# kujason/monopsr

Hardware: AMD Instinct MI355X
Metric: instance-crops/sec (fwd+Chamfer) (higher is better)
Workload: dtype f32; 1 GPU; BASELINE cfg3: batch=256/GPU synthetic 48x48 crops -> ResNet-101 trunk(block3, os4) + squash/map-decoder/xyz + heads fwd, + 1024-pt nn_distance Chamfer fwd/bwd; batch_per_gpu=256, global_batch=256, points=1024, streams_per_gpu=1

## Files before the change

monopsr_amd/csrc/internal.h:

```cpp
#pragma once
#include <hip/hip_runtime.h>

#include <atomic>
#include <cstddef>

#include "monopsr_hip.h"

namespace mpsr {

char *error_buffer();
extern thread_local int t_call_math;
extern thread_local int t_call_wino_policy;

int conv2d(const float *x, int B, int H, int W, int C, const float *w, const float *bias, const float *residual,
           float *y, int N, int KH, int KW, int dilation, int relu, int split_k, float *ws, size_t ws_floats,
           hipStream_t stream);
size_t conv_scratch_floats(long long M, int N);
bool conv2d_takes_winograd4(int B, int H, int W, int C, int N, const float *ws, size_t ws_floats);
bool conv2d_takes_winograd3(int B, int H, int W, int C, int N, int KH, int KW, int dilation, int split_k, const float *ws,
                            size_t ws_floats);
bool conv2d_takes_pointwise(long long M, int C, int N, int KH, int KW, int split_k);
int conv2d_winograd_choice(int B, int H, int W, int C, int N, int KH, int KW, int dilation, bool residual, int split_k,
                           const float *ws, size_t ws_floats);

int conv3x3_narrow(const float *x, int B, int H, int W, int C, const float *w, const float *bias, int relu, float *y,
                   int N, hipStream_t s, int in_c8);
bool conv3x3_narrow_takes_mfma(const float *x, int B, int H, int W, int C, int N, const float *w);
int resize_bilinear_c8(const float *in, int B, int H, int W, int C, int OH, int OW, int align_corners, float *out,
                       hipStream_t s);

size_t winograd_scratch_floats(int C, int N);
bool winograd_applies(int H, int W, int C, int N);
bool winograd_applies_dilated(int H, int W, int C, int N, int dilation);
int conv3x3_winograd(const float *x, int B, int H, int W, int C, const float *w, const float *bias, int relu, float *y,
                     int N, float *ws, size_t ws_floats, hipStream_t s, int dilation);
extern std::atomic<int> g_wino_waves;

size_t winograd4_scratch_floats(int C, int N);
bool winograd4_applies(int H, int W, int C, int N);
int conv3x3_winograd4(const float *x, int B, int H, int W, int C, const float *w, const float *bias, int relu,
                      float *y, int N, float *ws, size_t ws_floats, hipStream_t s, int in_c8, int out_c8, float *part,
                      size_t part_floats);
size_t winograd4_split_floats(int B, int H, int W, int N);
extern std::atomic<int> g_wino4_split;

size_t winograd3_scratch_floats(int C, int N);
bool winograd3_applies(int H, int W, int C, int dilation);
double winograd3_executed_flops(int B, int H, int C, int N, int dilation);
int winograd3_form(int B, int H, int W, int C, int N, int dilation);
int winograd3_filter_form(int B, int H, int W, int C, int N, int dilation);
int conv3x3_winograd3(const float *x, int B, int H, int W, int C, const float *w, const float *bias, int relu,
                      float *y, int N, int dilation, float *ws, size_t ws_floats, hipStream_t s,
                      const float *mask = nullptr);
struct FilterTailJob {
    const float *w = nullptr;
    float *u = nullptr;
    int N = 0, C = 0;
    int form = 0;
};
extern thread_local FilterTailJob g_filter_tail_job;
extern thread_local FilterTailJob g_filter_tail_done;
struct FilterCacheSlot {
    const float *w = nullptr;
    float *u = nullptr;
    size_t floats = 0;
    bool ready = false;
    int *tag = nullptr;
    bool holds(int kind)
    {
        const bool ok = ready && (!tag || *tag == kind);
        if (tag) *tag = kind;
        return ok;
    }
};
enum { FILTER_FORM_WINO4 = 1, FILTER_FORM_WINO3 = 2, FILTER_FORM_UPCONV = 3, FILTER_FORM_WINO3Z = 4, FILTER_FORM_WINO2 = 5 };
extern thread_local FilterCacheSlot g_filter_cache_slot;

bool winograd3w_applies(int B, int H, int W, int C, int N, int dilation);
long long winograd3w_workgroups(int B, int N, int dilation);
int launch_winograd3w(const float *x, int B, int H, int W, int C, const float *u, const float *bias, int relu, float *y,
                      int N, int dilation, hipStream_t s, const float *mask);

// ... 42 lines not shown
```

monopsr_amd/csrc/network.hip:

```cpp
#include <atomic>
#include <vector>

#include "common.h"

static std::atomic<int> g_decoder_c8{1};
extern "C" void mpsr_debug_set_decoder_c8(int on) { g_decoder_c8 = on; }
static std::atomic<int> g_decoder_upconv{1};
extern "C" void mpsr_debug_set_decoder_upconv(int on) { g_decoder_upconv = on; }

namespace {

struct Arena {
    char *base;
    size_t size, used = 0;
    bool ok = true;
    Arena(void *p, size_t n) : base(static_cast<char *>(p)), size(n) {}
    float *floats(size_t n)
    {
        const size_t bytes = mpsr::align_up(n * sizeof(float), 256);
        if (used + bytes > size) {
            ok = false;
            return nullptr;
        }
        float *r = reinterpret_cast<float *>(base + used);
// ... 91 lines not shown
                              int n_layers, float *out, void *workspace, size_t workspace_bytes, mpsr_stream_t stream)
{
    return mpsr_trunk_fwd_ex(img, B, H, W, blob, layers, n_layers, out, workspace, workspace_bytes, nullptr, stream);
}

extern "C" int mpsr_trunk_fwd_ex(const float *img, int B, int H, int W, const float *blob, const mpsr_layer *layers,
                                 int n_layers, float *out, void *workspace, size_t workspace_bytes,
                                 const mpsr_net_opts *opts, mpsr_stream_t stream)
{
    MPSR_REQUIRE(B >= 0 && H >= 7 && W >= 7, "trunk_fwd: bad input shape (B=%d H=%d W=%d)", B, H, W);
    if (opts) {
        MPSR_REQUIRE(opts->math >= 0 && opts->math <= MPSR_CALL_MATH_BF16X3, "%s: unknown opts.math %d", "trunk_fwd", opts->math);
        MPSR_REQUIRE(opts->winograd_policy >= 0 && opts->winograd_policy <= MPSR_CALL_WINOGRAD_ACCURATE,
                     "%s: unknown opts.winograd_policy %d", "trunk_fwd", opts->winograd_policy);
    }
    mpsr::CallOptsGuard call_opts(opts ? opts->math : 0, opts ? opts->winograd_policy : 0);
    MPSR_REQUIRE(n_layers == MPSR_TRUNK_LAYERS, "trunk_fwd: expected %d layer records, got %d", MPSR_TRUNK_LAYERS,
                 n_layers);
    if (B == 0) return MPSR_OK;
    MPSR_REQUIRE(img && blob && layers && out && workspace, "trunk_fwd: null pointer");
    hipStream_t s = mpsr::as_stream(stream);
    const TrunkDims d = trunk_dims(H, W);
    const size_t Mr = (size_t)B * d.OH * d.OW, Mp = (size_t)B * d.PH * d.PW;
    const mpsr_layer &root = layers[0];
    MPSR_REQUIRE(root.kh == 1 && root.kw == 1 && root.cin >= 147 && root.cin % 32 == 0,
                 "trunk_fwd: layer 0 must be the root as a 1x1 layer over im2col columns (cin=%d)", root.cin);
    int cmax = 0, bmax = 0;
    for (int i = 1; i < n_layers; ++i) {
        if (layers[i].kh == 3 && layers[i].cout > bmax) bmax = layers[i].cout;
        if (layers[i].cout > cmax) cmax = layers[i].cout;
    }
    Arena ar(workspace, workspace_bytes);
    float *cols = ar.floats(Mr * root.cin);
    float *rootout = ar.floats(Mr * root.cout);
    float *pooled = ar.floats(Mp * root.cout);
    float *ping = ar.floats(Mp * cmax), *pong = ar.floats(Mp * cmax), *scut = ar.floats(Mp * cmax);
    float *t1 = ar.floats(Mp * bmax), *t2 = ar.floats(Mp * bmax);
    const size_t skn = mpsr::conv_scratch_floats((long long)(Mr > Mp ? Mr : Mp), cmax > 1024 ? cmax : 1024);
    float *sk = ar.floats(skn);
    if (!ar.ok)
        return mpsr::fail(MPSR_ERR_WORKSPACE, "trunk_fwd: workspace %zu bytes too small (see mpsr_trunk_workspace_bytes)",
                          workspace_bytes);

    int rc;
    struct TailJobGuard {
        ~TailJobGuard()
        {
            mpsr::g_filter_tail_job = mpsr::FilterTailJob();
            mpsr::g_filter_tail_done = mpsr::FilterTailJob();
            mpsr::g_filter_cache_slot = mpsr::FilterCacheSlot();
        }
    } tail_job_guard;
    FilterCache cache(opts);
    if ((rc = mpsr_im2col_root(img, B, H, W, cols, root.cin, stream))) return rc;
    if ((rc = run_layer(blob, root, cols, B, d.OH, d.OW, nullptr, rootout, 0, sk, skn, s))) return rc;
    if ((rc = mpsr_max_pool(rootout, B, d.OH, d.OW, root.cout, 3, 2, 1, pooled, stream))) return rc;

    const float *cur = pooled;
    int cur_c = root.cout;
    int li = 1;
    for (int blk = 0; blk < 3; ++blk) {
        for (int u = 0; u < kTrunkUnits[blk]; ++u) {
            const bool last = (blk == 2 && u == kTrunkUnits[blk] - 1);
            const float *residual = cur;
            if (u == 0) {
                const mpsr_layer &S = layers[li++];
                MPSR_REQUIRE(S.kh == 1 && S.cin == cur_c && !S.relu, "trunk_fwd: record %d is not a shortcut", li - 1);
                if ((rc = run_layer(blob, S, cur, B, d.PH, d.PW, nullptr, scut, 0, sk, skn, s))) return rc;
                residual = scut;
            }
            const mpsr_layer &c1 = layers[li], &c2 = layers[li + 1], &c3 = layers[li + 2];
            li += 3;
            MPSR_REQUIRE(c1.kh == 1 && c1.cin == cur_c && c2.kh == 3 && c2.cin == c1.cout && c3.kh == 1 &&
                             c3.cin == c2.cout && (u == 0 || c3.cout == cur_c),
                         "trunk_fwd: records %d..%d do not form a bottleneck unit", li - 3, li - 1);
            float *dst = last ? out : (cur == ping ? pong : ping);
            float *uslice = cache.take(c2);
            const int c2i = (int)(&c2 - layers);
            const int fform = mpsr::winograd3_filter_form(B, d.PH, d.PW, c2.cin, c2.cout, c2.dilation);
            const bool cached_u = uslice && cache.valid && (!cache.tags || cache.tags[c2i] == fform);
            if (!cached_u &&
                mpsr::conv2d_takes_pointwise((long long)B * d.PH * d.PW, c1.cin, c1.cout, 1, 1, 0) &&
                mpsr::conv2d_takes_winograd3(B, d.PH, d.PW, c2.cin, c2.cout, c2.kh, c2.kw, c2.dilation, 0, sk, skn)) {
                mpsr::g_filter_tail_job.w = blob + c2.w_off;
                mpsr::g_filter_tail_job.u = uslice ? uslice : sk;
                mpsr::g_filter_tail_job.N = c2.cout;
                mpsr::g_filter_tail_job.C = c2.cin;
                mpsr::g_filter_tail_job.form = fform == mpsr::FILTER_FORM_WINO3Z ? 1 : 0;
            }
            if ((rc = run_layer(blob, c1, cur, B, d.PH, d.PW, nullptr, t1, 0, sk, skn, s))) return rc;
            mpsr::g_filter_tail_job = mpsr::FilterTailJob();
            cache.offer(blob + c2.w_off, uslice, c2, c2i);
            rc = run_layer(blob, c2, t1, B, d.PH, d.PW, nullptr, t2, 0, sk, skn, s);
            mpsr::g_filter_cache_slot = mpsr::FilterCacheSlot();
            if (rc) return rc;
            if ((rc = run_layer(blob, c3, t2, B, d.PH, d.PW, residual, dst, 0, sk, skn, s))) return rc;
            cur = dst;
            cur_c = c3.cout;
        }
    }
    return MPSR_OK;
}


namespace {
struct DecoderChoice {
    bool c8, up1, up2, xyz_c8;
};
DecoderChoice decoder_choice(int B, int fh, int fw, int mh, int mw, const mpsr_layer *L, const float *blob, bool feat_map,
// ... 398 lines not shown
```

monopsr_amd/csrc/upconv.hip:

```cpp
#include <atomic>

#include "common.h"

namespace {

using f32x2 = __attribute__((ext_vector_type(2))) float;
using f32x4 = __attribute__((ext_vector_type(4))) float;
constexpr int PART = 1152;
constexpr size_t kGatherLdsBytes = 80 * 1024;

__global__ __launch_bounds__(256) void upconv_weights_kernel(const float *__restrict__ g, int N, int C, float *__restrict__ wp)
{
    const long long i = (long long)blockIdx.x * 256 + threadIdx.x;
    const int c4 = C / 4;
    if (i >= (long long)9 * N * c4) return;
    const int j = (int)(i / c4), q = (int)(i - (long long)j * c4);
    const int blk = j / 72, r = j - blk * 72, t = r >> 3, n = blk * 8 + (r & 7);
    reinterpret_cast<float4 *>(wp)[i] = reinterpret_cast<const float4 *>(g + ((size_t)n * 9 + t) * C)[q];
}

struct UpcParams {
    const float *z, *bias;
    float *y;
    size_t part_stride;
    int B, h, w, H, W, N, relu;
    int RB, cap;
    mpsr::FastDiv capdiv;
    float hscale, wscale;
};

constexpr int kPf = 8;
std::atomic<int> g_upconv_band{0};

template <bool OUT_C8>
__global__ __launch_bounds__(512) void upconv_gather_kernel(const UpcParams p)
{
    extern __shared__ __attribute__((aligned(16))) float4 src4[];
    const int tid = threadIdx.x, nthr = blockDim.x;
    const int nblk = p.N >> 3;
    const int xcd = blockIdx.x & 7, jx = blockIdx.x >> 3;
    const int bq = jx / nblk, blk = jx - bq * nblk, b = bq * 8 + xcd;
    if (b >= p.B) return;
    const int lpr = 2 * p.W, rpp = nthr / lpr;
    const int rr = tid / lpr, l = tid - rr * lpr, x = l >> 1, half = l & 1;
    const int n0 = blk * 8;
    const int rowf4 = p.w * 18;
    auto slot = [&](int r) __attribute__((always_inline)) { return r - p.cap * mpsr::fdiv(r, p.capdiv); };
    const float *zp = p.z + (size_t)(blk >> 4) * p.part_stride + (size_t)(blk & 15) * 72 + (size_t)b * p.h * p.w * PART;
    const int lgroups = nthr / 18, lgrp = tid / 18, lpiece = tid - lgrp * 18;
    const bool loader = lgrp < lgroups;
    const int lrow0 = lgrp / p.w, lcol0 = lgrp - lrow0 * p.w;
    const int drow = lgroups / p.w, dcol = lgroups - drow * p.w;
    f32x4 pf[kPf];
    auto issue = [&](int ra, int npix, int first) __attribute__((always_inline)) {
#pragma unroll
        for (int j = 0; j < kPf; ++j) {
            const int pix = first + lgrp + j * lgroups;
            const bool live = loader && pix < npix;
            pf[j] = *reinterpret_cast<const f32x4 *>(live ? zp + ((size_t)ra * p.w + pix) * PART + 4 * lpiece : zp);
        }
    };
    auto commit = [&](int ra, int npix, int first, int &row, int &col) __attribute__((always_inline)) {
#pragma unroll
        for (int j = 0; j < kPf; ++j) {
            const int pix = first + lgrp + j * lgroups;
            if (loader && pix < npix)
                reinterpret_cast<f32x4 *>(src4)[slot(ra + row) * rowf4 + col * 18 + lpiece] = pf[j];
            row += drow;
            col += dcol;
            if (col >= p.w) {
                col -= p.w;
                ++row;
            }
        }
    };

    auto band_rows = [&](int k, int &lo, int &hi) __attribute__((always_inline)) {
        const int y0 = k * p.RB, yl = min(y0 + p.RB, p.H) - 1;
        lo = (int)floorf((float)max(y0 - 1, 0) * p.hscale);
        hi = min((int)floorf((float)min(yl + 1, p.H - 1) * p.hscale) + 1, p.h - 1);
    };
    int co[3][2];
    float wx[3][2];
#pragma unroll
    for (int d = 0; d < 3; ++d) {
        const int qx = x + d - 1;
        const bool vx = qx >= 0 && qx < p.W;
        const float sx = (float)min(max(qx, 0), p.W - 1) * p.wscale;
        const int c0 = (int)floorf(sx), c1 = min(c0 + 1, p.w - 1);
        const float lx = sx - (float)c0;
        co[d][0] = c0 * 18 + half;
        co[d][1] = c1 * 18 + half;
        wx[d][0] = vx ? 1.f - lx : 0.f;
        wx[d][1] = vx ? lx : 0.f;
    }
    const float4 bias4 = p.bias ? *reinterpret_cast<const float4 *>(p.bias + n0 + 4 * half) : make_float4(0.f, 0.f, 0.f, 0.f);

    const int nbands = (p.H + p.RB - 1) / p.RB;
    int lo, hi;
    band_rows(0, lo, hi);
    {
        const int npix = (hi - lo + 1) * p.w;
        int row = lrow0, col = lcol0;
        for (int first = 0; first < npix; first += kPf * lgroups) {
            issue(lo, npix, first);
            commit(lo, npix, first, row, col);
        }
    }
    __syncthreads();
    for (int k = 0; k < nbands; ++k) {
        int nlo = 0, nhi = hi;
        if (k + 1 < nbands) band_rows(k + 1, nlo, nhi);
        const int nnew = (nhi - hi) * p.w;
        issue(hi + 1, nnew, 0);
        const int y0 = k * p.RB, ylast = min(y0 + p.RB, p.H) - 1;
        for (int y = y0 + rr; y <= ylast; y += rpp) {
            int ro[3][2];
            float wy[3][2];
#pragma unroll
            for (int d = 0; d < 3; ++d) {
                const int qy = y + d - 1;
                const bool vy = qy >= 0 && qy < p.H;
                const float sy = (float)min(max(qy, 0), p.H - 1) * p.hscale;
                const int r0 = (int)floorf(sy), r1 = min(r0 + 1, p.h - 1);
                const float ly = sy - (float)r0;
                ro[d][0] = slot(r0) * rowf4;
                ro[d][1] = slot(r1) * rowf4;
                wy[d][0] = vy ? 1.f - ly : 0.f;
                wy[d][1] = vy ? ly : 0.f;
            }
            f32x2 a01 = {bias4.x, bias4.y}, a23 = {bias4.z, bias4.w};
#pragma unroll
            for (int dy = 0; dy < 3; ++dy)
#pragma unroll
                for (int dx = 0; dx < 3; ++dx) {
                    const int t2 = 2 * (dy * 3 + dx);
#pragma unroll
                    for (int a = 0; a < 2; ++a)
#pragma unroll
                        for (int c = 0; c < 2; ++c) {
                            const float wgt = wy[dy][a] * wx[dx][c];
                            const float4 v = src4[ro[dy][a] + co[dx][c] + t2];
                            const f32x2 w2 = {wgt, wgt};
                            a01 = __builtin_elementwise_fma(w2, f32x2{v.x, v.y}, a01);
                            a23 = __builtin_elementwise_fma(w2, f32x2{v.z, v.w}, a23);
                        }
                }
            float4 acc = make_float4(a01.x, a01.y, a23.x, a23.y);
            if (p.relu) {
                acc.x = fmaxf(acc.x, 0.f);
                acc.y = fmaxf(acc.y, 0.f);
                acc.z = fmaxf(acc.z, 0.f);
                acc.w = fmaxf(acc.w, 0.f);
            }
            float *o = OUT_C8 ? p.y + ((((size_t)b * (p.N / 8) + blk) * p.H + y) * p.W + x) * 8 + 4 * half
                              : p.y + (((size_t)b * p.H + y) * p.W + x) * p.N + n0 + 4 * half;
            *reinterpret_cast<float4 *>(o) = acc;
        }
        if (k + 1 == nbands) break;
        __syncthreads();
        {
            int row = lrow0, col = lcol0;
            commit(hi + 1, nnew, 0, row, col);
        }
        __syncthreads();
        hi = nhi;
    }
}

constexpr int kGtMax = 8;
constexpr int kGtPf = 6;
constexpr int kGtItemsA = 6, kGtItemsB = 8;

struct UpcGradParams {
    const float *dy;
    float *dz;
    int B, h, w, H, W, N, rows_max, cap;
    float hscale, wscale;
};

__global__ __launch_bounds__(256) void upconv_gather_t_kernel(const UpcGradParams p)
{
    extern __shared__ __attribute__((aligned(16))) float4 g4[];
    const int tid = threadIdx.x;
    const int grp = blockIdx.x, b = blockIdx.y;
    const int rowq = p.W * 8;
    float4 *V = g4 + (size_t)p.cap * rowq;
    int *xq = reinterpret_cast<int *>(V + (size_t)3 * rowq);
    float *xw = reinterpret_cast<float *>(xq + p.w * kGtMax);
    int *xc = reinterpret_cast<int *>(xw + p.w * kGtMax);
    int *yq = xc + ((p.w + 3) & ~3);
    float *yw = reinterpret_cast<float *>(yq + p.h * kGtMax);
    int *yc = reinterpret_cast<int *>(yw + p.h * kGtMax);
    int *ylo = yc + p.h, *yhi = ylo + p.h;
    for (int t = tid; t < p.h + p.w; t += 256) {
        const bool row = t < p.h;
        const int sv = row ? t : t - p.h, n_in = row ? p.h : p.w, n_out = row ? p.H : p.W;
        const float scale = row ? p.hscale : p.wscale;
        const int q_lo = max((int)floorf((float)(sv - 1) / scale) - 1, 0), q_hi = min((int)ceilf((float)(sv + 1) / scale) + 1, n_out - 1);
        int *oq = row ? yq + sv * kGtMax : xq + sv * kGtMax;
        float *ow = row ? yw + sv * kGtMax : xw + sv * kGtMax;
        int c = 0, lo = n_out, hi = -1;
        for (int q = q_lo; q <= q_hi; ++q) {
            const float sq = (float)q * scale;
            const int r0 = (int)floorf(sq), r1 = min(r0 + 1, n_in - 1);
            const float l = sq - (float)r0;
            if ((r0 == sv || r1 == sv) && c < kGtMax) {
                oq[c] = q;
                ow[c] = (r0 == sv ? 1.f - l : 0.f) + (r1 == sv ? l : 0.f);
                ++c;
                lo = min(lo, q);
                hi = max(hi, q);
            }
        }
        if (row) {
            yc[sv] = c;
            ylo[sv] = c ? max(lo - 1, 0) : 0;
            yhi[sv] = c ? min(hi + 1, p.H - 1) : -1;
        } else {
// ... 98 lines not shown
            const int4 q4 = *reinterpret_cast<const int4 *>(xq + sx * kGtMax);
            const float4 w4 = *reinterpret_cast<const float4 *>(xw + sx * kGtMax);
            const float4 *row = V + b_v[k];
            const int px0 = q4.x - dx, px1 = q4.y - dx, px2 = q4.z - dx, px3 = q4.w - dx;
            const bool ok0 = nx > 0 && px0 >= 0 && px0 < p.W, ok1 = nx > 1 && px1 >= 0 && px1 < p.W;
            const bool ok2 = nx > 2 && px2 >= 0 && px2 < p.W, ok3 = nx > 3 && px3 >= 0 && px3 < p.W;
            const float4 v0 = row[(ok0 ? px0 : 0) * 8], v1 = row[(ok1 ? px1 : 0) * 8];
            const float4 v2 = row[(ok2 ? px2 : 0) * 8], v3 = row[(ok3 ? px3 : 0) * 8];
            f32x2 a01 = {0.f, 0.f}, a23 = {0.f, 0.f};
            auto acc = [&](float wv, const float4 &v) __attribute__((always_inline)) {
                const f32x2 w2_ = {wv, wv};
                a01 = __builtin_elementwise_fma(w2_, f32x2{v.x, v.y}, a01);
                a23 = __builtin_elementwise_fma(w2_, f32x2{v.z, v.w}, a23);
            };
            if (ok0) acc(w4.x, v0);
            if (ok1) acc(w4.y, v1);
            if (ok2) acc(w4.z, v2);
            if (ok3) acc(w4.w, v3);
            for (int kx = 4; kx < nx; ++kx) {
                const int px = xq[sx * kGtMax + kx] - dx;
                if (px < 0 || px >= p.W) continue;
                acc(xw[sx * kGtMax + kx], row[px * 8]);
            }
            *reinterpret_cast<float4 *>(dzrow + b_out[k]) = make_float4(a01.x, a01.y, a23.x, a23.y);
        }
        if (more) commit(have + 1, next_hi);
        have = next_hi;
        __syncthreads();
    }
}

__global__ __launch_bounds__(256) void upconv_weights_t_kernel(const float *__restrict__ g, int N, int C, float *__restrict__ wt)
{
    const long long i = (long long)blockIdx.x * 256 + threadIdx.x;
    const int K = 9 * N;
    if (i >= (long long)C * K) return;
    const int c = (int)(i / K), j = (int)(i - (long long)c * K);
    const int blk = j / 72, r = j - blk * 72, t = r >> 3, n = blk * 8 + (r & 7);
    wt[i] = g[((size_t)n * 9 + t) * C + c];
}

__global__ __launch_bounds__(256) void upconv_fold_dw_kernel(const float *__restrict__ dwp, int N, int C, float *__restrict__ dw)
{
    const long long i = (long long)blockIdx.x * 256 + threadIdx.x;
    const int c4 = C / 4;
    if (i >= (long long)9 * N * c4) return;
    const int j = (int)(i / c4), q = (int)(i - (long long)j * c4);
    const int blk = j / 72, r = j - blk * 72, t = r >> 3, n = blk * 8 + (r & 7);
    float4 *d = reinterpret_cast<float4 *>(dw + ((size_t)n * 9 + t) * C) + q;
    const float4 a = *d, v = reinterpret_cast<const float4 *>(dwp)[i];
    *d = make_float4(a.x + v.x, a.y + v.y, a.z + v.z, a.w + v.w);
}

bool gather_geometry(int h, int w, int H, int W, float hscale, int *threads, int *RB, int *cap)
{
    if (2 * W > 512 || w < 1) return false;
    int rpp = 1;
    while (rpp * 2 <= 16 && rpp * 2 * 2 * W <= 512) rpp *= 2;
    const int nthr = rpp * 2 * W;
    if (nthr < 18) return false;
    int rb = rpp > 8 ? rpp : 8;
    if (g_upconv_band.load() > 0) {
        rb = (g_upconv_band.load() + rpp - 1) / rpp * rpp;
    } else if ((size_t)h * w * 288 <= kGatherLdsBytes * 3 / 5) {
        rb = (H + rpp - 1) / rpp * rpp;
    }
    int rows = 0, add = 0, prev_hi = -1;
    for (int k = 0; k * rb < H; ++k) {
        const int y0 = k * rb, yl = (y0 + rb < H ? y0 + rb : H) - 1;
        const int lo = (int)floorf((float)(y0 - 1 > 0 ? y0 - 1 : 0) * hscale);
        int hi = (int)floorf((float)(yl + 1 < H - 1 ? yl + 1 : H - 1) * hscale) + 1;
        if (hi > h - 1) hi = h - 1;
        if (hi - lo + 1 > rows) rows = hi - lo + 1;
        if (k > 0 && hi - prev_hi > add) add = hi - prev_hi;
        prev_hi = hi;
    }
    if (add * w > kPf * (nthr / 18)) return false;
    const int c = rows;
    if ((size_t)c * w * 288 > kGatherLdsBytes) return false;
    *threads = nthr;
    *RB = rb;
    *cap = c;
    return true;
}

}

static std::atomic<int> g_upconv_chunk_mb{0};
extern "C" void mpsr_debug_set_upconv_chunk_mb(int mb) { g_upconv_chunk_mb = mb > 0 ? mb : 0; }
extern "C" void mpsr_debug_set_upconv_band(int rows) { g_upconv_band = rows > 0 ? rows : 0; }

namespace mpsr {

static bool upconv_geometry_ok(int h, int w, int OH, int OW, int align_corners)
{
    int t, rb, cap;
    const float hs = (align_corners && OH > 1) ? (float)(h - 1) / (float)(OH - 1) : (float)h / (float)OH;
    return gather_geometry(h, w, OH, OW, hs, &t, &rb, &cap);
}

size_t upconv_weight_floats(int C, int N) { return (size_t)9 * N * C; }
size_t upconv_z_floats(long long Msrc, int N) { return (size_t)Msrc * 9 * (size_t)N; }

bool upconv_applies(int B, int h, int w, int C, int OH, int OW, int N, int align_corners)
{
    const long long M = (long long)B * h * w;
    return B > 0 && h >= 1 && w >= 1 && OH >= 1 && OW >= 1 && N >= 128 && N % 128 == 0 && C % 4 == 0 &&
           pointwise_applies(M, C, PART) && upconv_geometry_ok(h, w, OH, OW, align_corners) && B <= 65535 &&
           (long long)B * OH * OW * N * 4 < 0x7fffffffffLL;
}

int conv3x3_upsampled(const float *x, int B, int h, int w, int C, int OH, int OW, int align_corners, const float *g,
                      const float *bias, int relu, float *y, int N, int out_c8, float *z, size_t z_floats, float *ws,
                      size_t ws_floats, hipStream_t s)
{
    MPSR_REQUIRE(upconv_applies(B, h, w, C, OH, OW, N, align_corners), "conv3x3_upsampled: unsupported shape (B=%d %dx%dx%d -> %dx%dx%d)",
                 B, h, w, C, OH, OW, N);
    const long long M = (long long)B * h * w;
    if (!z || z_floats < upconv_z_floats(M, N))
        return fail(MPSR_ERR_WORKSPACE, "conv3x3_upsampled: z scratch holds %zu floats, needs %zu", z_floats,
                    upconv_z_floats(M, N));
    float *wp = ws;
    bool ready = false;
    if (g_filter_cache_slot.w == g && g_filter_cache_slot.u && g_filter_cache_slot.floats >= upconv_weight_floats(C, N)) {
        wp = g_filter_cache_slot.u;
        ready = g_filter_cache_slot.holds(FILTER_FORM_UPCONV);
    } else if (!ws || ws_floats < upconv_weight_floats(C, N)) {
        g_filter_cache_slot = FilterCacheSlot();
        return fail(MPSR_ERR_WORKSPACE, "conv3x3_upsampled: scratch holds %zu floats, needs %zu", ws_floats,
                    upconv_weight_floats(C, N));
    }
    g_filter_cache_slot = FilterCacheSlot();
    if (!ready) {
        const long long total = (long long)9 * N * (C / 4);
        hipLaunchKernelGGL(upconv_weights_kernel, dim3((unsigned)((total + 255) / 256)), dim3(256), 0, s, g, N, C, wp);
        MPSR_CHECK_LAUNCH("upconv_weights_kernel");
    }
    const int parts = N / 128;
    UpcParams p;
    p.bias = bias;
    p.part_stride = (size_t)M * PART;
    p.h = h; p.w = w; p.H = OH; p.W = OW; p.N = N; p.relu = relu;
    p.hscale = (align_corners && OH > 1) ? (float)(h - 1) / (float)(OH - 1) : (float)h / (float)OH;
    p.wscale = (align_corners && OW > 1) ? (float)(w - 1) / (float)(OW - 1) : (float)w / (float)OW;
    int threads = 0;
    if (!gather_geometry(h, w, OH, OW, p.hscale, &threads, &p.RB, &p.cap))
        return fail(MPSR_ERR_UNSUPPORTED, "conv3x3_upsampled: no gather geometry for a %dx%d -> %dx%d map", h, w, OH, OW);
    p.capdiv = make_fastdiv(p.cap);
    const size_t lds = (size_t)p.cap * w * 288;
    const int chunk_mb = g_upconv_chunk_mb.load();
    int bc = B;
    if (chunk_mb > 0) {
        const double per_image = (double)h * w * 9.0 * N * 4.0;
        bc = (int)((double)chunk_mb * 1048576.0 / per_image);
        bc = bc < 8 ? 8 : bc / 8 * 8;
        const int nch = ceil_div(B, bc);
        bc = ceil_div(ceil_div(B, nch), 8) * 8;
    }
    for (int b0 = 0; b0 < B; b0 += bc) {
        const int nb = B - b0 < bc ? B - b0 : bc;
        const size_t pix0 = (size_t)b0 * h * w;
        for (int pidx = 0; pidx < parts; ++pidx) {
            const int rc = conv1x1_pointwise(x + pix0 * C, (long long)nb * h * w, C, wp + (size_t)pidx * PART * C, nullptr,
                                             nullptr, 0, z + (size_t)pidx * M * PART + pix0 * PART, PART, s);
            if (rc) return rc;
        }
        p.z = z + pix0 * PART;
        p.y = y + (size_t)b0 * OH * OW * N;
        p.B = nb;
        const dim3 grid((unsigned)(8 * ceil_div(nb, 8) * (N / 8)));
        if (out_c8) {
            MPSR_CHECK_HIP(hipFuncSetAttribute(reinterpret_cast<const void *>(upconv_gather_kernel<true>),
                                               hipFuncAttributeMaxDynamicSharedMemorySize, (int)lds));
            hipLaunchKernelGGL(upconv_gather_kernel<true>, grid, dim3(threads), lds, s, p);
        } else {
            MPSR_CHECK_HIP(hipFuncSetAttribute(reinterpret_cast<const void *>(upconv_gather_kernel<false>),
                                               hipFuncAttributeMaxDynamicSharedMemorySize, (int)lds));
            hipLaunchKernelGGL(upconv_gather_kernel<false>, grid, dim3(threads), lds, s, p);
        }
        MPSR_CHECK_LAUNCH("upconv_gather_kernel");
    }
    return MPSR_OK;
}

}

namespace mpsr {

static int gather_t_rows(int h, int OH, float hscale)
{
    int most = 1;
    for (int sy = 0; sy < h; ++sy) {
        int lo = OH, hi = -1;
        for (int q = 0; q < OH; ++q) {
            const float sq = (float)q * hscale;
            const int r0 = (int)floorf(sq), r1 = r0 + 1 < h - 1 ? r0 + 1 : h - 1;
            if (r0 == sy || r1 == sy) {
                lo = q < lo ? q : lo;
                hi = q > hi ? q : hi;
            }
        }
        if (hi >= lo) {
            const int a = lo - 1 > 0 ? lo - 1 : 0, b = hi + 1 < OH - 1 ? hi + 1 : OH - 1;
            most = b - a + 1 > most ? b - a + 1 : most;
        }
    }
    return most;
}
static int gather_t_cap(int rows)
{
    int cap = 1;
    while (cap < rows) cap *= 2;
    return cap;
}
static size_t gather_t_lds_bytes(int rows, int h, int w, int OW)
{
    return (size_t)(gather_t_cap(rows) + 3) * OW * 128 + (size_t)w * (kGtMax * 8 + 4) + 16 + (size_t)h * (kGtMax * 8 + 12);
}
static int gather_t_new_rows(int h, int OH, float hscale)
{
    int most = 0, have = -1;
    for (int sy = 0; sy < h; ++sy) {
        int hi = -1;
        for (int q = 0; q < OH; ++q) {
            const float sq = (float)q * hscale;
            const int r0 = (int)floorf(sq), r1 = r0 + 1 < h - 1 ? r0 + 1 : h - 1;
            if (r0 == sy || r1 == sy) hi = q;
        }
        if (hi >= 0) {
            const int e = hi + 1 < OH - 1 ? hi + 1 : OH - 1;
            if (have >= 0 && e - have > most) most = e - have;
            if (e > have) have = e;
// ... 114 lines not shown
```

Measured before the change: 19490 crops/s.

## Fuse stem im2col, 7x7 conv, ReLU and max-pool into one MFMA kernel

Adds a single kernel that stages an input window in LDS, computes the 7x7 stride-2 stem conv with fp32 MFMA, applies bias and ReLU, and max-pools into shared memory using integer atomic max on the non-negative float bits. The trunk calls it when the shape and math mode match, and otherwise falls back to the im2col plus GEMM plus pool path. This removes the im2col column buffer and the full-resolution conv output round trips through global memory, along with two kernel launches. The cost is LDS atomics, recomputed halo pixels between tiles, and a narrow set of shapes where the fused path applies.

```diff
diff --git a/monopsr_amd/csrc/internal.h b/monopsr_amd/csrc/internal.h
--- a/monopsr_amd/csrc/internal.h
+++ b/monopsr_amd/csrc/internal.h
@@ -28,6 +28,9 @@
 bool conv3x3_narrow_takes_mfma(const float *x, int B, int H, int W, int C, int N, const float *w);
 int resize_bilinear_c8(const float *in, int B, int H, int W, int C, int OH, int OW, int align_corners, float *out,
                        hipStream_t s);
+
+bool stem_fused_applies(int B, int H, int W, int kpad, int cout, int relu, const float *w, const float *out);
+int stem_fused(const float *img, int B, int H, int W, const float *w, const float *bias, float *out, hipStream_t s);
 
 size_t winograd_scratch_floats(int C, int N);
 bool winograd_applies(int H, int W, int C, int N);
diff --git a/monopsr_amd/csrc/network.hip b/monopsr_amd/csrc/network.hip
--- a/monopsr_amd/csrc/network.hip
+++ b/monopsr_amd/csrc/network.hip
@@ -167,9 +167,14 @@
         }
     } tail_job_guard;
     FilterCache cache(opts);
-    if ((rc = mpsr_im2col_root(img, B, H, W, cols, root.cin, stream))) return rc;
-    if ((rc = run_layer(blob, root, cols, B, d.OH, d.OW, nullptr, rootout, 0, sk, skn, s))) return rc;
-    if ((rc = mpsr_max_pool(rootout, B, d.OH, d.OW, root.cout, 3, 2, 1, pooled, stream))) return rc;
+    if (mpsr::stem_fused_applies(B, H, W, root.cin, root.cout, root.relu, blob + root.w_off, pooled)) {
+        if ((rc = mpsr::stem_fused(img, B, H, W, blob + root.w_off, root.b_off >= 0 ? blob + root.b_off : nullptr, pooled, s)))
+            return rc;
+    } else {
+        if ((rc = mpsr_im2col_root(img, B, H, W, cols, root.cin, stream))) return rc;
+        if ((rc = run_layer(blob, root, cols, B, d.OH, d.OW, nullptr, rootout, 0, sk, skn, s))) return rc;
+        if ((rc = mpsr_max_pool(rootout, B, d.OH, d.OW, root.cout, 3, 2, 1, pooled, stream))) return rc;
+    }
 
     const float *cur = pooled;
     int cur_c = root.cout;
diff --git a/monopsr_amd/csrc/stem.hip b/monopsr_amd/csrc/stem.hip
--- /dev/null
+++ b/monopsr_amd/csrc/stem.hip
@@ -0,0 +1,179 @@
+#include "common.h"
+
+namespace {
+
+using f32x16 = __attribute__((ext_vector_type(16))) float;
+
+constexpr int KPAD = 160, KREAL = 147, NOUT = 64;
+constexpr int TP = 12;
+constexpr int CT = 2 * TP + 1;
+constexpr int WIN = 2 * CT + 5;
+constexpr int WSTRIDE = WIN * 3;
+constexpr int WFLOATS = WIN * WSTRIDE;
+constexpr int WPAD = 16;
+constexpr int THREADS = 512;
+constexpr int STAGE = (WFLOATS + WPAD + THREADS - 1) / THREADS;
+
+struct StemParams {
+    const float *x, *w, *bias;
+    float *y;
+    int H, W, OH, OW, PH, PW;
+    int pt, pl;
+};
+
+constexpr int koff(int k) { return (k / 21) * WSTRIDE + k % 21; }
+
+__global__ __launch_bounds__(THREADS) void stem_fused_kernel(const StemParams p)
+{
+    __shared__ __attribute__((aligned(16))) float win[WFLOATS + WPAD];
+    __shared__ __attribute__((aligned(16))) int pooled[TP * TP * NOUT];
+
+    const int tid = threadIdx.x, lane = tid & 63, wave = tid >> 6;
+    const int b = blockIdx.z, py0 = blockIdx.y * TP, px0 = blockIdx.x * TP;
+    const int cy0 = max(2 * py0 - p.pt, 0), cy1 = min(2 * (py0 + TP - 1) - p.pt + 3, p.OH);
+    const int cx0 = max(2 * px0 - p.pl, 0), cx1 = min(2 * (px0 + TP - 1) - p.pl + 3, p.OW);
+    const int ch = cy1 - cy0, cw = cx1 - cx0, npix = ch * cw;
+    const float inv_cw = 1.0f / (float)cw;
+
+    {
+        const int iy0 = 2 * cy0 - 3, ic0 = (2 * cx0 - 3) * 3;
+        const int wr = 2 * ch + 5, wc = (2 * cw + 5) * 3, W3 = p.W * 3;
+        const float *xb = p.x + (size_t)b * p.H * W3;
+        float v[STAGE];
+#pragma unroll
+        for (int it = 0; it < STAGE; ++it) {
+            const int e = tid + it * THREADS;
+            const int r = e / WSTRIDE, c = e - r * WSTRIDE;
+            const int iy = iy0 + r, ic = ic0 + c;
+            const bool ok = (r < wr) & (c < wc) & (iy >= 0) & (iy < p.H) & (ic >= 0) & (ic < W3);
+            v[it] = 0.f;
+            if (ok) v[it] = xb[iy * W3 + ic];
+        }
+#pragma unroll
+        for (int it = 0; it < STAGE; ++it) {
+            const int e = tid + it * THREADS;
+            if (e < WFLOATS + WPAD) win[e] = v[it];
+        }
+        for (int i = tid; i < TP * TP * NOUT; i += THREADS) pooled[i] = 0;
+    }
+
+    const int nt = wave & 1, h = lane >> 5;
+    const int n = nt * 32 + (lane & 31);
+    float bw[KPAD / 2];
+    {
+        const float4 *wrow = reinterpret_cast<const float4 *>(p.w + n * KPAD + 4 * h);
+#pragma unroll
+        for (int j = 0; j < KPAD / 8; ++j) {
+            const float4 t = wrow[2 * j];
+            bw[4 * j] = t.x; bw[4 * j + 1] = t.y; bw[4 * j + 2] = t.z; bw[4 * j + 3] = t.w;
+        }
+    }
+    const float bias = p.bias ? p.bias[n] : 0.f;
+    __syncthreads();
+
+    const int mtiles = (npix + 31) >> 5;
+    for (int mt = wave >> 1; mt < mtiles; mt += 4) {
+        int q = mt * 32 + (lane & 31);
+        q = q < npix ? q : 0;
+        const int ly = (int)(((float)q + 0.5f) * inv_cw), lx = q - ly * cw;
+        const int pix = ly * (2 * WSTRIDE) + lx * 6;
+        const float *pa = win + pix + 4 * h, *pb = win + pix + (4 + WSTRIDE - 21) * h;
+        f32x16 acc;
+#pragma unroll
+        for (int e = 0; e < 16; ++e) acc[e] = 0.f;
+#pragma unroll
+        for (int j = 0; j < KPAD / 8; ++j) {
+#pragma unroll
+            for (int s = 0; s < 4; ++s) {
+                const int k0 = 8 * j + s;
+                float a = 0.f;
+                if (k0 < KREAL) {
+                    a = (k0 % 21 >= 17 && k0 + 4 < KREAL ? pb : pa)[koff(k0)];
+                    if (k0 + 4 >= KREAL) a = h ? 0.f : a;
+                }
+                acc = __builtin_amdgcn_mfma_f32_32x32x2f32(a, bw[4 * j + s], acc, 0, 0, 0);
+            }
+        }
+        asm volatile("s_nop 15\n\ts_nop 7" : "+a"(acc));
+
+#pragma unroll
+        for (int e = 0; e < 16; ++e) {
+            const int qe = mt * 32 + (e & 3) + 8 * (e >> 2) + 4 * h;
+            float v = acc[e];
+            if (p.bias) v += bias;
+            v = fmaxf(v, 0.f);
+            const int bits = __float_as_int(v);
+            if (qe < npix && bits > 0) {
+                const int ey = (int)(((float)qe + 0.5f) * inv_cw), ex = qe - ey * cw;
+                const int qy = cy0 + ey + p.pt - 2 * py0, qx = cx0 + ex + p.pl - 2 * px0;
+                const int ty = qy >> 1, tx = qx >> 1;
+                const bool y0 = ty < TP, y1 = !(qy & 1) && ty >= 1;
+                const bool x0 = tx < TP, x1 = !(qx & 1) && tx >= 1;
+                int *cell = pooled + (ty * TP + tx) * NOUT + n;
+                if (y0 && x0) __hip_atomic_fetch_max(cell, bits, __ATOMIC_RELAXED, __HIP_MEMORY_SCOPE_WORKGROUP);
+                if (y0 && x1) __hip_atomic_fetch_max(cell - NOUT, bits, __ATOMIC_RELAXED, __HIP_MEMORY_SCOPE_WORKGROUP);
+                if (y1 && x0)
+                    __hip_atomic_fetch_max(cell - TP * NOUT, bits, __ATOMIC_RELAXED, __HIP_MEMORY_SCOPE_WORKGROUP);
+                if (y1 && x1)
+                    __hip_atomic_fetch_max(cell - (TP + 1) * NOUT, bits, __ATOMIC_RELAXED, __HIP_MEMORY_SCOPE_WORKGROUP);
+            }
+        }
+    }
+    __syncthreads();
+
+    for (int i = tid; i < TP * TP * (NOUT / 4); i += THREADS) {
+        const int cell = i / (NOUT / 4), c4 = i - cell * (NOUT / 4);
+        const int ty = cell / TP, tx = cell - ty * TP;
+        const int py = py0 + ty, px = px0 + tx;
+        if (py < p.PH && px < p.PW)
+            *reinterpret_cast<int4 *>(p.y + (((size_t)b * p.PH + py) * p.PW + px) * NOUT + c4 * 4) =
+                *reinterpret_cast<const int4 *>(&pooled[cell * NOUT + c4 * 4]);
+    }
+}
+
+inline bool aligned16(const void *p) { return (reinterpret_cast<uintptr_t>(p) & 15) == 0; }
+
+}
+
+namespace mpsr {
+
+bool stem_fused_applies(int B, int H, int W, int kpad, int cout, int relu, const float *w, const float *out)
+{
+    if (B < 1 || B > 65535 || H < 7 || W < 7 || kpad != KPAD || cout != NOUT || !relu) return false;
+    if ((t_call_math >= 0 ? t_call_math : mpsr_get_conv_math()) != MPSR_MATH_FP32) return false;
+    if (!aligned16(w) || !aligned16(out) || (long long)H * W * 3 >= 0x7fffffffLL) return false;
+    const int OH = (H - 1) / 2 + 1;
+    return ceil_div((OH + 1) / 2, TP) <= 65535;
+}
+
+int stem_fused(const float *img, int B, int H, int W, const float *w, const float *bias, float *out, hipStream_t s)
+{
+    StemParams p;
+    p.x = img; p.w = w; p.bias = bias; p.y = out;
+    p.H = H; p.W = W;
+    p.OH = (H + 6 - 7) / 2 + 1;
+    p.OW = (W + 6 - 7) / 2 + 1;
+    p.PH = ceil_div(p.OH, 2);
+    p.PW = ceil_div(p.OW, 2);
+    const int th = (p.PH - 1) * 2 + 3 - p.OH, tw = (p.PW - 1) * 2 + 3 - p.OW;
+    p.pt = (th > 0 ? th : 0) / 2;
+    p.pl = (tw > 0 ? tw : 0) / 2;
+    const dim3 grid((unsigned)ceil_div(p.PW, TP), (unsigned)ceil_div(p.PH, TP), (unsigned)B);
+    hipLaunchKernelGGL(stem_fused_kernel, grid, dim3(THREADS), 0, s, p);
+    MPSR_CHECK_LAUNCH("stem_fused_kernel");
+    return MPSR_OK;
+}
+
+}
+
+extern "C" int mpsr_debug_stem_fwd(const float *img, int B, int H, int W, const float *w, const float *bias, int kpad,
+                                   int cout, int relu, float *out, mpsr_stream_t stream)
+{
+    MPSR_REQUIRE(B >= 0 && H >= 7 && W >= 7, "stem_fwd: bad input shape (B=%d H=%d W=%d)", B, H, W);
+    if (B == 0) return MPSR_OK;
+    MPSR_REQUIRE(img && w && out, "stem_fwd: null pointer");
+    if (!mpsr::stem_fused_applies(B, H, W, kpad, cout, relu, w, out))
+        return mpsr::fail(MPSR_ERR_UNSUPPORTED, "stem_fwd: not a shape of the fused stem (kpad=%d cout=%d relu=%d)", kpad,
+                          cout, relu);
+    return mpsr::stem_fused(img, B, H, W, w, bias, out, mpsr::as_stream(stream));
+}
```

Result: no change. 19570 crops/s (median of 6 runs) (+0.4%).

## Split upconv gather into separable horizontal then vertical passes with staged rows

Applied to the files above, without the earlier changes.

The fused bilinear-upsample plus 3x3 conv gather now runs in two passes. A horizontal pass interpolates staged source rows per dx tap into an LDS ring of per-output-column rows, and the vertical pass blends only two rows per dy, replacing 36 float4 LDS reads per output with 6 plus the horizontal work. Source rows are streamed through a small staging buffer with prefetch depth set by a new geometry parameter, instead of keeping whole source bands in LDS. This cuts per-output LDS reads and FMAs, but adds more __syncthreads per row and a new WIDE template path, and it changes LDS sizing.

```diff
diff --git a/monopsr_amd/csrc/upconv.hip b/monopsr_amd/csrc/upconv.hip
--- a/monopsr_amd/csrc/upconv.hip
+++ b/monopsr_amd/csrc/upconv.hip
@@ -24,18 +24,18 @@
     float *y;
     size_t part_stride;
     int B, h, w, H, W, N, relu;
-    int RB, cap;
+    int RB, cap, stg;
     mpsr::FastDiv capdiv;
     float hscale, wscale;
 };
 
-constexpr int kPf = 8;
+constexpr int kPf = 4;
 std::atomic<int> g_upconv_band{0};
 
-template <bool OUT_C8>
+template <bool OUT_C8, bool WIDE = false>
 __global__ __launch_bounds__(512) void upconv_gather_kernel(const UpcParams p)
 {
-    extern __shared__ __attribute__((aligned(16))) float4 src4[];
+    extern __shared__ __attribute__((aligned(16))) float4 lds4[];
     const int tid = threadIdx.x, nthr = blockDim.x;
     const int nblk = p.N >> 3;
     const int xcd = blockIdx.x & 7, jx = blockIdx.x >> 3;
@@ -45,6 +45,9 @@
     const int rr = tid / lpr, l = tid - rr * lpr, x = l >> 1, half = l & 1;
     const int n0 = blk * 8;
     const int rowf4 = p.w * 18;
+    const int hrow4 = 3 * lpr;
+    float4 *hr = lds4;
+    float4 *zs = lds4 + (size_t)p.cap * hrow4;
     auto slot = [&](int r) __attribute__((always_inline)) { return r - p.cap * mpsr::fdiv(r, p.capdiv); };
     const float *zp = p.z + (size_t)(blk >> 4) * p.part_stride + (size_t)(blk & 15) * 72 + (size_t)b * p.h * p.w * PART;
     const int lgroups = nthr / 18, lgrp = tid / 18, lpiece = tid - lgrp * 18;
@@ -60,12 +63,12 @@
             pf[j] = *reinterpret_cast<const f32x4 *>(live ? zp + ((size_t)ra * p.w + pix) * PART + 4 * lpiece : zp);
         }
     };
-    auto commit = [&](int ra, int npix, int first, int &row, int &col) __attribute__((always_inline)) {
+    auto commit = [&](int npix) __attribute__((always_inline)) {
+        int row = lrow0, col = lcol0;
 #pragma unroll
         for (int j = 0; j < kPf; ++j) {
-            const int pix = first + lgrp + j * lgroups;
-            if (loader && pix < npix)
-                reinterpret_cast<f32x4 *>(src4)[slot(ra + row) * rowf4 + col * 18 + lpiece] = pf[j];
+            const int pix = lgrp + j * lgroups;
+            if (loader && pix < npix) reinterpret_cast<f32x4 *>(zs)[row * rowf4 + col * 18 + lpiece] = pf[j];
             row += drow;
             col += dcol;
             if (col >= p.w) {
@@ -75,10 +78,18 @@
         }
     };
 
-    auto band_rows = [&](int k, int &lo, int &hi) __attribute__((always_inline)) {
-        const int y0 = k * p.RB, yl = min(y0 + p.RB, p.H) - 1;
-        lo = (int)floorf((float)max(y0 - 1, 0) * p.hscale);
-        hi = min((int)floorf((float)min(yl + 1, p.H - 1) * p.hscale) + 1, p.h - 1);
+    auto commit_row = [&](int npix, int first) __attribute__((always_inline)) {
+#pragma unroll
+        for (int j = 0; j < kPf; ++j) {
+            const int pix = first + lgrp + j * lgroups;
+            if (loader && pix < npix) reinterpret_cast<f32x4 *>(zs)[pix * 18 + lpiece] = pf[j];
+        }
+    };
+    constexpr bool wide = WIDE;
+
+    auto band_hi = [&](int k) __attribute__((always_inline)) {
+        const int yl = min(k * p.RB + p.RB, p.H) - 1;
+        return min((int)floorf((float)min(yl + 1, p.H - 1) * p.hscale) + 1, p.h - 1);
     };
     int co[3][2];
     float wx[3][2];
@@ -89,30 +100,56 @@
         const float sx = (float)min(max(qx, 0), p.W - 1) * p.wscale;
         const int c0 = (int)floorf(sx), c1 = min(c0 + 1, p.w - 1);
         const float lx = sx - (float)c0;
-        co[d][0] = c0 * 18 + half;
-        co[d][1] = c1 * 18 + half;
+        co[d][0] = c0 * 18 + 2 * d + half;
+        co[d][1] = c1 * 18 + 2 * d + half;
         wx[d][0] = vx ? 1.f - lx : 0.f;
         wx[d][1] = vx ? lx : 0.f;
     }
     const float4 bias4 = p.bias ? *reinterpret_cast<const float4 *>(p.bias + n0 + 4 * half) : make_float4(0.f, 0.f, 0.f, 0.f);
 
     const int nbands = (p.H + p.RB - 1) / p.RB;
-    int lo, hi;
-    band_rows(0, lo, hi);
-    {
-        const int npix = (hi - lo + 1) * p.w;
-        int row = lrow0, col = lcol0;
-        for (int first = 0; first < npix; first += kPf * lgroups) {
-            issue(lo, npix, first);
-            commit(lo, npix, first, row, col);
-        }
-    }
-    __syncthreads();
+    int have = -1;
+    int pn = wide ? 0 : min(band_hi(0) + 1, p.stg);
+    if (pn > 0) issue(0, pn * p.w, 0);
     for (int k = 0; k < nbands; ++k) {
-        int nlo = 0, nhi = hi;
-        if (k + 1 < nbands) band_rows(k + 1, nlo, nhi);
-        const int nnew = (nhi - hi) * p.w;
-        issue(hi + 1, nnew, 0);
+        const int bhi = band_hi(k);
+        while (have < bhi) {
+            if (wide) {
+                for (int first = 0; first < p.w; first += kPf * lgroups) {
+                    issue(have + 1, p.w, first);
+                    commit_row(p.w, first);
+                }
+                pn = 1;
+            } else {
+                if (pn == 0) {
+                    pn = min(bhi - have, p.stg);
+                    issue(have + 1, pn * p.w, 0);
+                }
+                commit(pn * p.w);
+            }
+            __syncthreads();
+            const int c0 = have + 1, cn = pn;
+            have += pn;
+            const int tgt = (have < bhi || k + 1 == nbands) ? bhi : band_hi(k + 1);
+            pn = wide ? 0 : min(tgt - have, p.stg);
+            if (pn > 0) issue(have + 1, pn * p.w, 0);
+            for (int q = rr; q < 3 * cn; q += rpp) {
+                const int rl = q / 3, dy = q - 3 * rl;
+                const float4 *zr = zs + rl * rowf4 + 6 * dy;
+                f32x2 a01 = {0.f, 0.f}, a23 = {0.f, 0.f};
+#pragma unroll
+                for (int dx = 0; dx < 3; ++dx)
+#pragma unroll
+                    for (int c = 0; c < 2; ++c) {
+                        const float4 v = zr[co[dx][c]];
+                        const f32x2 w2 = {wx[dx][c], wx[dx][c]};
+                        a01 = __builtin_elementwise_fma(w2, f32x2{v.x, v.y}, a01);
+                        a23 = __builtin_elementwise_fma(w2, f32x2{v.z, v.w}, a23);
+                    }
+                hr[(slot(c0 + rl) * 3 + dy) * lpr + l] = make_float4(a01.x, a01.y, a23.x, a23.y);
+            }
+            __syncthreads();
+        }
         const int y0 = k * p.RB, ylast = min(y0 + p.RB, p.H) - 1;
         for (int y = y0 + rr; y <= ylast; y += rpp) {
             int ro[3][2];
@@ -124,8 +161,8 @@
                 const float sy = (float)min(max(qy, 0), p.H - 1) * p.hscale;
                 const int r0 = (int)floorf(sy), r1 = min(r0 + 1, p.h - 1);
                 const float ly = sy - (float)r0;
-                ro[d][0] = slot(r0) * rowf4;
-                ro[d][1] = slot(r1) * rowf4;
+                ro[d][0] = (slot(r0) * 3 + d) * lpr + l;
+                ro[d][1] = (slot(r1) * 3 + d) * lpr + l;
                 wy[d][0] = vy ? 1.f - ly : 0.f;
                 wy[d][1] = vy ? ly : 0.f;
             }
@@ -133,18 +170,11 @@
 #pragma unroll
             for (int dy = 0; dy < 3; ++dy)
 #pragma unroll
-                for (int dx = 0; dx < 3; ++dx) {
-                    const int t2 = 2 * (dy * 3 + dx);
-#pragma unroll
-                    for (int a = 0; a < 2; ++a)
-#pragma unroll
-                        for (int c = 0; c < 2; ++c) {
-                            const float wgt = wy[dy][a] * wx[dx][c];
-                            const float4 v = src4[ro[dy][a] + co[dx][c] + t2];
-                            const f32x2 w2 = {wgt, wgt};
-                            a01 = __builtin_elementwise_fma(w2, f32x2{v.x, v.y}, a01);
-                            a23 = __builtin_elementwise_fma(w2, f32x2{v.z, v.w}, a23);
-                        }
+                for (int a = 0; a < 2; ++a) {
+                    const float4 v = hr[ro[dy][a]];
+                    const f32x2 w2 = {wy[dy][a], wy[dy][a]};
+                    a01 = __builtin_elementwise_fma(w2, f32x2{v.x, v.y}, a01);
+                    a23 = __builtin_elementwise_fma(w2, f32x2{v.z, v.w}, a23);
                 }
             float4 acc = make_float4(a01.x, a01.y, a23.x, a23.y);
             if (p.relu) {
@@ -157,14 +187,6 @@
                               : p.y + (((size_t)b * p.H + y) * p.W + x) * p.N + n0 + 4 * half;
             *reinterpret_cast<float4 *>(o) = acc;
         }
-        if (k + 1 == nbands) break;
-        __syncthreads();
-        {
-            int row = lrow0, col = lcol0;
-            commit(hi + 1, nnew, 0, row, col);
-        }
-        __syncthreads();
-        hi = nhi;
     }
 }
 
@@ -369,7 +391,7 @@
     *d = make_float4(a.x + v.x, a.y + v.y, a.z + v.z, a.w + v.w);
 }
 
-bool gather_geometry(int h, int w, int H, int W, float hscale, int *threads, int *RB, int *cap)
+bool gather_geometry(int h, int w, int H, int W, float hscale, int *threads, int *RB, int *cap, int *stage)
 {
     if (2 * W > 512 || w < 1) return false;
     int rpp = 1;
@@ -382,7 +404,7 @@
     } else if ((size_t)h * w * 288 <= kGatherLdsBytes * 3 / 5) {
         rb = (H + rpp - 1) / rpp * rpp;
     }
-    int rows = 0, add = 0, prev_hi = -1;
+    int rows = 0, add = 0, first = 0, prev_hi = -1;
     for (int k = 0; k * rb < H; ++k) {
         const int y0 = k * rb, yl = (y0 + rb < H ? y0 + rb : H) - 1;
         const int lo = (int)floorf((float)(y0 - 1 > 0 ? y0 - 1 : 0) * hscale);
@@ -390,14 +412,21 @@
         if (hi > h - 1) hi = h - 1;
         if (hi - lo + 1 > rows) rows = hi - lo + 1;
         if (k > 0 && hi - prev_hi > add) add = hi - prev_hi;
+        if (k == 0) first = hi + 1;
         prev_hi = hi;
     }
-    if (add * w > kPf * (nthr / 18)) return false;
-    const int c = rows;
-    if ((size_t)c * w * 288 > kGatherLdsBytes) return false;
+    const int per_chunk = kPf * (nthr / 18) / w > 1 ? kPf * (nthr / 18) / w : 1;
+    if ((size_t)rows * w * 288 > kGatherLdsBytes || add * w > 8 * (nthr / 18)) return false;
+    const size_t ring = (size_t)rows * 3 * W * 32, zrow = (size_t)w * 288;
+    const size_t budget = ring + zrow <= kGatherLdsBytes * 3 / 5 ? kGatherLdsBytes * 3 / 5 : kGatherLdsBytes;
+    int stg = first > add ? first : add;
+    if (stg > per_chunk) stg = per_chunk;
+    while (stg > 1 && ring + stg * zrow > budget) --stg;
+    if (ring + stg * zrow > kGatherLdsBytes) return false;
     *threads = nthr;
     *RB = rb;
-    *cap = c;
+    *cap = rows;
+    *stage = stg;
     return true;
 }
 
@@ -411,9 +440,9 @@
 
 static bool upconv_geometry_ok(int h, int w, int OH, int OW, int align_corners)
 {
-    int t, rb, cap;
+    int t, rb, cap, stg;
     const float hs = (align_corners && OH > 1) ? (float)(h - 1) / (float)(OH - 1) : (float)h / (float)OH;
-    return gather_geometry(h, w, OH, OW, hs, &t, &rb, &cap);
+    return gather_geometry(h, w, OH, OW, hs, &t, &rb, &cap, &stg);
 }
 
 size_t upconv_weight_floats(int C, int N) { return (size_t)9 * N * C; }
@@ -461,10 +490,10 @@
     p.hscale = (align_corners && OH > 1) ? (float)(h - 1) / (float)(OH - 1) : (float)h / (float)OH;
     p.wscale = (align_corners && OW > 1) ? (float)(w - 1) / (float)(OW - 1) : (float)w / (float)OW;
     int threads = 0;
-    if (!gather_geometry(h, w, OH, OW, p.hscale, &threads, &p.RB, &p.cap))
+    if (!gather_geometry(h, w, OH, OW, p.hscale, &threads, &p.RB, &p.cap, &p.stg))
         return fail(MPSR_ERR_UNSUPPORTED, "conv3x3_upsampled: no gather geometry for a %dx%d -> %dx%d map", h, w, OH, OW);
     p.capdiv = make_fastdiv(p.cap);
-    const size_t lds = (size_t)p.cap * w * 288;
+    const size_t lds = (size_t)p.cap * 3 * OW * 32 + (size_t)p.stg * w * 288;
     const int chunk_mb = g_upconv_chunk_mb.load();
     int bc = B;
     if (chunk_mb > 0) {
@@ -486,15 +515,21 @@
         p.y = y + (size_t)b0 * OH * OW * N;
         p.B = nb;
         const dim3 grid((unsigned)(8 * ceil_div(nb, 8) * (N / 8)));
+#define MPSR_UPC(...)                                                                                                 \
+    do {                                                                                                              \
+        MPSR_CHECK_HIP(hipFuncSetAttribute(reinterpret_cast<const void *>(upconv_gather_kernel<__VA_ARGS__>),         \
+                                           hipFuncAttributeMaxDynamicSharedMemorySize, (int)lds));                    \
+        hipLaunchKernelGGL((upconv_gather_kernel<__VA_ARGS__>), grid, dim3(threads), lds, s, p);                      \
+    } while (0)
+        const bool wide = p.stg * w > kPf * (threads / 18);
         if (out_c8) {
-            MPSR_CHECK_HIP(hipFuncSetAttribute(reinterpret_cast<const void *>(upconv_gather_kernel<true>),
-                                               hipFuncAttributeMaxDynamicSharedMemorySize, (int)lds));
-            hipLaunchKernelGGL(upconv_gather_kernel<true>, grid, dim3(threads), lds, s, p);
+            if (wide) MPSR_UPC(true, true);
+            else MPSR_UPC(true, false);
         } else {
-            MPSR_CHECK_HIP(hipFuncSetAttribute(reinterpret_cast<const void *>(upconv_gather_kernel<false>),
-                                               hipFuncAttributeMaxDynamicSharedMemorySize, (int)lds));
-            hipLaunchKernelGGL(upconv_gather_kernel<false>, grid, dim3(threads), lds, s, p);
-        }
+            if (wide) MPSR_UPC(false, true);
+            else MPSR_UPC(false, false);
+        }
+#undef MPSR_UPC
         MPSR_CHECK_LAUNCH("upconv_gather_kernel");
     }
     return MPSR_OK;
```

New measurement: 19500 crops/s before, 19700 crops/s after (median of 6 runs). 1.1% higher.
